# JNP-Solutions/Slacken

Hardware: AMD Instinct MI355X
Metric: classify_throughput_150bp_standard224scale (higher is better)
Workload: dtype u64

## Files before the change

### slacken_amd/csrc/build.hip

```cpp
#include <hip/hip_runtime.h>

#include "engine.h"

namespace slk {

namespace {

constexpr int BW = 4;

__device__ int insert_merge(const TableBuild &t, const int32_t *parents, int32_t ntax, uint64_t key, int32_t taxon, int &max_d) {
  const uint64_t h = fmix64(key);
  if (!shard_keeps(t, h)) return 0;
  uint32_t home;
  uint64_t rem_hi;
  table_slot(t.g, h, home, rem_hi);
  const unsigned long long tmask = (1ULL << t.g.taxon_bits) - 1;
  for (int d = 0; d <= t.disp_limit; d++) {
    unsigned long long *bucket = (unsigned long long *)(t.cells + ((uint64_t)table_bucket(t.g, home, (uint32_t)d) * CELLS));
    const unsigned long long tag = rem_hi | (uint64_t)d;
    const unsigned long long val = (tag << t.g.taxon_bits) | (uint32_t)taxon;
    unsigned long long first = 0;
    for (int c = 0; c < CELLS; c++) {
      unsigned long long cur = __hip_atomic_load(&bucket[c], __ATOMIC_RELAXED, __HIP_MEMORY_SCOPE_AGENT);
      if (cur == 0) {
        unsigned long long old = atomicCAS(&bucket[c], 0ULL, val);
        if (old == 0) {
          max_d = max(max_d, d);
          return 1;
        }
        cur = old;
      }
      if (c == 0) first = cur;
      if (cell_tag(t.g, cur) == tag) {
        for (;;) {
          int32_t old_taxon = (int32_t)(cur & tmask);
          int32_t merged = tax_lca(parents, ntax, old_taxon, taxon);
          if (merged == old_taxon) return 0;
          unsigned long long want = (cur & ~tmask) | (uint32_t)merged;
          unsigned long long prev = atomicCAS(&bucket[c], cur, want);
          if (prev == cur) return 0;
          cur = prev;
        }
      }
    }
    if (t.g.flag && !(first & t.g.flag)) atomicOr(&bucket[0], (unsigned long long)t.g.flag);
  }
  return -1;
}

struct BuildLds {
  uint64_t q_key[BW][128];
  int32_t q_tax[BW][128];
};

__device__ __forceinline__ int code_of(uint32_t c) {
  const uint32_t VM = (1u << 1) | (1u << 3) | (1u << 7) | (1u << 20) | (1u << 21);
  bool ok = ((c & 0xC0) == 0x40) && ((VM >> (c & 31)) & 1);
  uint32_t t = (c >> 1) & 3;
  t ^= t >> 1;
  return ok ? (int)t : 5;
}

__global__ void __launch_bounds__(BW * 64) build_kernel(ScanParams P, TableBuild T, const int32_t *__restrict__ parents,
                                                        int32_t ntax, const uint8_t *__restrict__ bases, uint64_t total_bases,
                                                        const uint64_t *__restrict__ chunk_start,
                                                        const uint32_t *__restrict__ chunk_len,
                                                        const int32_t *__restrict__ chunk_taxon, uint64_t nchunks) {
  extern __shared__ uint64_t ring[];
  __shared__ BuildLds L;
  const uint32_t tid = threadIdx.x, lane = tid & 63;
  const uint32_t wib = __builtin_amdgcn_readfirstlane(tid >> 6);
  const uint32_t stride = BW * 64;
  const int w = P.w, k = P.k, m = P.m;
  const uint64_t c = (uint64_t)blockIdx.x * stride + tid;
  const uint32_t len = c < nchunks ? chunk_len[c] : 0;
  const uint64_t start = c < nchunks ? chunk_start[c] : 0;
  const int32_t taxon = c < nchunks ? chunk_taxon[c] : 0;
  uint32_t maxlen = len;
// ... 151 lines not shown
```

### slacken_amd/csrc/engine.h

```cpp
#pragma once
#include <hip/hip_runtime.h>
#include <stdint.h>

namespace slk {

struct ScanParams {
  int32_t k, m, w;
  int32_t canonical;
  int32_t sh;
  uint64_t xmask;
  uint64_t smask;
  uint64_t keep;
};

constexpr int WIDE_MAXW = 4;
struct WideParams {
  int32_t k, m, w, canonical;
  int32_t W;
  int32_t last_sh;
  uint64_t xmask[WIDE_MAXW];
  uint64_t smask[WIDE_MAXW];
};
struct WideTable {
  uint64_t *keys;
// ... 14 lines not shown
                              const int32_t *span_meta, const uint64_t *out_offsets, void *out, int64_t *out_keys, hipStream_t s);
void launch_wide_probe(const WideTable &t, int W, const uint64_t *offsets, const uint64_t *mate_offsets, uint64_t R,
                       const uint64_t *span_keys, const int32_t *span_meta, const int32_t *span_count, int32_t *span_taxon,
                       hipStream_t s);

#ifndef SLK_BUCKET_CELLS
#define SLK_BUCKET_CELLS 8
#endif
constexpr int CELLS = SLK_BUCKET_CELLS;
constexpr int LPB = CELLS / 2;
constexpr int BUCKET_SHIFT = CELLS == 16 ? 7 : 6;
static_assert(CELLS == 8 || CELLS == 16, "buckets of 64 or 128 bytes");
struct TableGeom {
  uint64_t nbuckets;
  uint64_t rem_mask;
  uint64_t flag;
  int32_t q;
  int32_t taxon_bits;
  int32_t disp_bits;
  int32_t pad;
};
__host__ __device__ __forceinline__ void table_slot(const TableGeom &g, uint64_t h, uint32_t &home, uint64_t &rem_hi) {
  const uint32_t x = (uint32_t)(h >> (64 - g.q));
  const uint64_t prod = (g.nbuckets >> 32) != 0 ? (uint64_t)x << 32 : (uint64_t)x * (uint32_t)g.nbuckets;
  home = (uint32_t)(prod >> g.q);
  const uint64_t extra = (prod & ((1ULL << g.q) - 1)) >= g.nbuckets ? 1 : 0;
  rem_hi = ((h & g.rem_mask) | (extra << (64 - g.q))) << g.disp_bits;
}
__host__ __device__ __forceinline__ uint32_t table_bucket(const TableGeom &g, uint32_t home, uint32_t d) {
  const uint64_t b = (uint64_t)home + d;
  return (uint32_t)(b >= g.nbuckets ? b - g.nbuckets : b);
}
__host__ __device__ __forceinline__ uint64_t cell_tag(const TableGeom &g, uint64_t cell) { return (cell & ~g.flag) >> g.taxon_bits; }
__host__ __device__ inline uint64_t table_hash_of(const TableGeom &g, uint32_t home, uint64_t rem) {
  const uint64_t extra = rem >> (64 - g.q);
  const uint64_t num = (uint64_t)home << g.q;
  const uint64_t x = (num + g.nbuckets - 1) / g.nbuckets + extra;
  return (x << (64 - g.q)) | (rem & g.rem_mask);
}
struct TableView {
  const uint64_t *cells;
  TableGeom g;
  int32_t max_disp;
  const int32_t *to_orig;
};
__device__ __forceinline__ int32_t ext_taxon(const TableView &T, int32_t t) { return (T.to_orig != nullptr && t > 0) ? T.to_orig[t] : t; }

__host__ __device__ inline uint64_t fmix64(uint64_t x) {
  x ^= x >> 33; x *= 0xff51afd7ed558ccdULL;
  x ^= x >> 33; x *= 0xc4ceb9fe1a85ec53ULL;
  x ^= x >> 33;
  return x;
}

__device__ __forceinline__ int32_t tax_parent(const int32_t *parents, int32_t ntax, int32_t t) {
  return ((uint32_t)t < (uint32_t)ntax) ? parents[t] : 0;
}

__device__ inline int32_t tax_lca(const int32_t *parents, int32_t ntax, int32_t a, int32_t b) {
  if (a == 0 || b == 0) return b == 0 ? a : b;
  if (a == b) return a;
  int da = 0, db = 0;
  for (int32_t x = a; x != 0; x = tax_parent(parents, ntax, x)) da++;
  for (int32_t y = b; y != 0; y = tax_parent(parents, ntax, y)) db++;
  for (; da > db; da--) a = tax_parent(parents, ntax, a);
  for (; db > da; db--) b = tax_parent(parents, ntax, b);
// ... 184 lines not shown
```

### slacken_amd/csrc/fused.hip

```cpp
#include "engine.h"

#include <cstdlib>

namespace slk {

constexpr int FW = 4;
constexpr int SPAN_CAP = 128;
constexpr int MAP_CAP = 128;
constexpr int32_t MAP_EMPTY = -1;

struct __attribute__((aligned(16))) RingLds {
  uint32_t fwd_ring[32 + 4];
  uint32_t rc_ring[32 + 4];
};
struct __attribute__((aligned(16))) WaveLds {
  uint64_t span_key[SPAN_CAP];
  int32_t span_meta[SPAN_CAP];
  uint64_t stash[128];
  int32_t result[64];
  int32_t map_key[MAP_CAP];
  int32_t map_cnt[MAP_CAP];
};

__device__ __forceinline__ void wave_sync() {
// ... 130 lines not shown
  int32_t flag = meta_flag(meta);
  bool seq = (lane < cnt) && flag == 1;
  uint64_t h = fmix64(key);
  uint32_t home;
  uint64_t rem_hi;
  table_slot(T.g, h, home, rem_hi);
  ulonglong2 st;
  st.x = home;
  st.y = seq ? rem_hi : NO_TAG;
  ((ulonglong2 *)L->stash)[lane] = st;
  L->result[lane] = 0;
  wave_sync();
  const int g = lane / LPB, c = lane % LPB;
  const uint64_t tmask = (1ULL << T.g.taxon_bits) - 1;
  const uint32_t gmask = (1u << LPB) - 1;
  const char *cellbase = (const char *)T.cells + c * 16;
  uint32_t more = 0;
  {
    ulonglong2 cell[LPB];
#pragma unroll
    for (int s = 0; s < LPB; s++) {
      ulonglong2 e = ((const ulonglong2 *)L->stash)[s * PG + g];
      cell[s] = make_ulonglong2(0, 0);
      if (e.y != NO_TAG) cell[s] = *(const ulonglong2 *)(cellbase + (e.x << BUCKET_SHIFT));
    }
#pragma unroll
    for (int s = 0; s < LPB; s++) {
      const uint64_t want = L->stash[2 * (s * PG + g) + 1];
      const bool act = want != NO_TAG;
      const bool e0 = cell[s].x == 0, e1 = cell[s].y == 0;
      const bool m0 = act && !e0 && cell_tag(T.g, cell[s].x) == want;
      const bool m1 = act && !e1 && cell_tag(T.g, cell[s].y) == want;
      if (m0 || m1) L->result[s * PG + g] = (int32_t)((m0 ? cell[s].x : cell[s].y) & tmask);
      const bool closed = T.g.flag != 0 && c == 0 && (cell[s].x & T.g.flag) == 0;
      const uint64_t B = __ballot(m0 || m1 || e0 || e1 || !act || closed);
      if (((B >> (g * LPB)) & gmask) == 0) more |= 1u << s;
    }
  }
  if (__ballot(more != 0) != 0) {
    for (int d = 1; d <= T.max_disp && __ballot(more != 0) != 0; d++) {
      for (int s = 0; s < LPB; s++) {
        const bool act = (more >> s) & 1;
        ulonglong2 cl = make_ulonglong2(0, 0);
        uint64_t want = 0;
        if (act) {
          ulonglong2 e = ((const ulonglong2 *)L->stash)[s * PG + g];
          want = e.y + (uint64_t)d;
          cl = *(const ulonglong2 *)(cellbase + ((uint64_t)table_bucket(T.g, (uint32_t)e.x, (uint32_t)d) << BUCKET_SHIFT));
        }
        const bool e0 = cl.x == 0, e1 = cl.y == 0;
        const bool m0 = act && !e0 && cell_tag(T.g, cl.x) == want;
        const bool m1 = act && !e1 && cell_tag(T.g, cl.y) == want;
        if (m0 || m1) L->result[s * PG + g] = (int32_t)((m0 ? cl.x : cl.y) & tmask);
        const bool closed = act && T.g.flag != 0 && c == 0 && (cl.x & T.g.flag) == 0;
        const uint64_t B = __ballot(act && (m0 || m1 || e0 || e1 || closed));
        if (act && ((B >> (g * LPB)) & gmask) != 0) more &= ~(1u << s);
      }
    }
  }
  wave_sync();
  int32_t taxon = L->result[lane];
  if (flag == 2) taxon = -1;
  else if (flag == 3) taxon = -2;
  return taxon;
}

__device__ __forceinline__ int char_code2(uint8_t c) {
  uint32_t x = ((uint32_t)(c & 0xDF)) - 0x41;
  switch (x) {
    case 0: return 0;
    case 2: return 1;
    case 6: return 2;
    case 0x13: return 3;
    case 0x14: return 3;
    default: return 5;
  }
}

__device__ int32_t lca_uniform(const int32_t *parents, int32_t ntax, int32_t a, int32_t b) {
  if (a == 0 || b == 0) return b == 0 ? a : b;
  for (int32_t y = b; y != 0; y = ((uint32_t)y < (uint32_t)ntax) ? parents[y] : 0)
    for (int32_t x = a; x != 0; x = ((uint32_t)x < (uint32_t)ntax) ? parents[x] : 0)
      if (x == y) return y;
  return 1;
}

__device__ __forceinline__ uint4 tax_node(const FusedArgs &A, int32_t t) {
// ... 790 lines not shown
```

### slacken_amd/csrc/kernels.hip

```cpp
#include "engine.h"

#include <algorithm>

namespace slk {


__global__ void __launch_bounds__(256) table_insert_kernel(TableBuild t, const int64_t *__restrict__ keys,
                                                           const int32_t *__restrict__ taxa, uint64_t n) {
  uint64_t i = (uint64_t)blockIdx.x * blockDim.x + threadIdx.x;
  uint64_t stride = (uint64_t)gridDim.x * blockDim.x;
  int n_ins = 0, n_dup = 0, n_ovf = 0, max_d = 0;
  for (; i < n; i += stride) {
    int32_t taxon = taxa[i];
    if (taxon == 0) continue;
    uint64_t h = fmix64((uint64_t)keys[i]);
    if (!shard_keeps(t, h)) continue;
    uint32_t home;
    uint64_t rem_hi;
    table_slot(t.g, h, home, rem_hi);
    bool done = false;
    for (int d = 0; d <= t.disp_limit && !done; d++) {
      unsigned long long *bucket = (unsigned long long *)(t.cells + ((uint64_t)table_bucket(t.g, home, (uint32_t)d) * CELLS));
      uint64_t tag = rem_hi | (uint64_t)d;
      unsigned long long val = (tag << t.g.taxon_bits) | (uint32_t)taxon;
      unsigned long long first = 0;
      for (int c = 0; c < CELLS && !done; c++) {
        unsigned long long cur = __hip_atomic_load(&bucket[c], __ATOMIC_RELAXED, __HIP_MEMORY_SCOPE_AGENT);
        if (cur == 0) {
          unsigned long long old = atomicCAS(&bucket[c], 0ULL, val);
          if (old == 0) {
            done = true;
            n_ins++;
            max_d = max(max_d, d);
            break;
          }
          cur = old;
        }
        if (c == 0) first = cur;
        if (cell_tag(t.g, cur) == tag) {
          done = true;
          n_dup++;
        }
      }
      if (!done && t.g.flag && !(first & t.g.flag)) atomicOr(&bucket[0], (unsigned long long)t.g.flag);
    }
    if (!done) n_ovf++;
  }
  for (int o = 32; o > 0; o >>= 1) {
    n_ins += __shfl_xor(n_ins, o);
    n_dup += __shfl_xor(n_dup, o);
    n_ovf += __shfl_xor(n_ovf, o);
    max_d = max(max_d, __shfl_xor(max_d, o));
  }
  if ((threadIdx.x & 63) == 0) {
    if (n_ins) atomicAdd(t.n_inserted, (unsigned long long)n_ins);
    if (n_dup) atomicAdd(t.n_duplicate, (unsigned long long)n_dup);
    if (n_ovf) atomicAdd(t.n_overflow, (unsigned long long)n_ovf);
    if (max_d) atomicMax(t.max_disp, max_d);
  }
}

__device__ __forceinline__ int32_t table_lookup(const TableView &t, uint64_t key) {
  uint64_t h = fmix64(key);
  uint32_t home;
  uint64_t rem_hi;
  table_slot(t.g, h, home, rem_hi);
  uint64_t tmask = (1ULL << t.g.taxon_bits) - 1;
  for (int d = 0; d <= t.max_disp; d++) {
    const ulonglong2 *b = (const ulonglong2 *)(t.cells + ((uint64_t)table_bucket(t.g, home, (uint32_t)d) * CELLS));
    uint64_t tag = rem_hi | (uint64_t)d;
    uint64_t cells[CELLS];
#pragma unroll
    for (int c = 0; c < LPB; c++) { ulonglong2 v = b[c]; cells[2 * c] = v.x; cells[2 * c + 1] = v.y; }
    bool has_empty = false;
    int32_t found = 0;
#pragma unroll
    for (int c = 0; c < CELLS; c++) {
      has_empty |= (cells[c] == 0);
      if (cells[c] != 0 && cell_tag(t.g, cells[c]) == tag) found = (int32_t)(cells[c] & tmask);
    }
    if (found) return found;
    if (has_empty) return 0;
    if (t.g.flag && !(cells[0] & t.g.flag)) return 0;
  }
  return 0;
}

__global__ void __launch_bounds__(256) table_lookup_kernel(TableView t, const int64_t *__restrict__ keys, uint64_t n,
                                                           int32_t *__restrict__ out) {
  uint64_t i = (uint64_t)blockIdx.x * blockDim.x + threadIdx.x;
  uint64_t stride = (uint64_t)gridDim.x * blockDim.x;
  for (; i < n; i += stride) out[i] = ext_taxon(t, table_lookup(t, (uint64_t)keys[i]));
}


__device__ __forceinline__ int char_code(uint8_t c) {
  if (c == '\n' || c == '\r') return 4;
  switch (c | 0x20) {
    case 'a': return 0;
    case 'c': return 1;
    case 'g': return 2;
    case 't': return 3;
    case 'u': return 3;
    default: return 5;
  }
}

struct SpanWriter {
  uint64_t *keys;
  int32_t *meta;
  uint64_t base;
  int32_t n;
  bool first;
  bool have_last;
  uint64_t last;

// ... 602 lines not shown
```

### slacken_amd/csrc/lane.hip

```cpp
#include "engine.h"

#include <algorithm>
#include <cstddef>
#include <cstdio>
#include <cstdlib>

namespace slk {

#ifndef SLK_LANE_LW
#define SLK_LANE_LW 4
#endif
constexpr int LW = SLK_LANE_LW;
constexpr int QCAP = 128;
#ifndef SLK_SBLK
#define SLK_SBLK 5
#endif
constexpr int SBLK = SLK_SBLK;
#ifndef SLK_OMAP
#define SLK_OMAP 12
#endif
constexpr int OMAP = SLK_OMAP;
constexpr int OMAP_CNT_BITS = 10;
constexpr uint32_t OMAP_CNT_MASK = (1u << OMAP_CNT_BITS) - 1;

struct __attribute__((aligned(16))) LaneLds {
  uint64_t q_key[QCAP];
  uint32_t q_meta[QCAP];
  uint64_t stash[128];
  uint32_t found[64];
  uint4 sbuf[(SBLK - 1) * 64];
  uint32_t omap[OMAP * 64];
  uint32_t o_flags[64];
  uint64_t rb[64];
  uint16_t q_ord[QCAP];
};

#ifdef SLK_TUNING
#define SLK_TUNE(...) __VA_ARGS__
#define SLK_TUNE_ON(bit) ((dbg & (bit)) != 0)
#else
#define SLK_TUNE(...)
#define SLK_TUNE_ON(bit) false
#endif

#ifndef SLK_PROBE_NT
#define SLK_PROBE_NT 0
#endif
__device__ __forceinline__ ulonglong2 SLK_PROBE_LOAD(const ulonglong2 *p) {
#if SLK_PROBE_NT
  ulonglong2 v;
  v.x = __builtin_nontemporal_load(&p->x);
  v.y = __builtin_nontemporal_load(&p->y);
  return v;
#else
  return *p;
#endif
}

__device__ __forceinline__ void lane_wave_sync() {
  __builtin_amdgcn_fence(__ATOMIC_RELEASE, "wavefront");
  __builtin_amdgcn_wave_barrier();
  __builtin_amdgcn_fence(__ATOMIC_ACQUIRE, "wavefront");
}
__device__ __forceinline__ uint64_t lmin64(uint64_t a, uint64_t b) { return a < b ? a : b; }

template <bool LONG>
__device__ __forceinline__ void fold_hit(LaneLds *L, uint32_t *ocnt, bool in, uint32_t meta, int32_t taxon) {
  if (in && taxon != 0) {
    const int owner = meta & 63;
    const int32_t kmers = (int32_t)((meta >> 7) & 0x1FFF);
    if (meta & 64) atomicAdd(&L->o_flags[owner], 1u);
    uint32_t slot = (uint32_t)(((uint64_t)((uint32_t)taxon * 0x9E3779B1u) * (uint32_t)OMAP) >> 32);
    int p = 0;
    if (LONG) {
      for (; p < OMAP; p++) {
// ... 19 lines not shown
__device__ __forceinline__ int probe_batch(LaneLds *L, uint32_t *ocnt, const TableView &T, int qhead, int qn, int cnt, int lane, int dbg,
                                           int32_t *hit_meta, int32_t *hit_taxon) {
  const uint64_t NO_TAG = ~0ULL;
  const bool in = lane < cnt;
  const int qi = (qhead + lane) & (QCAP - 1);
  const uint64_t key = L->q_key[qi];
  const uint32_t meta = L->q_meta[qi];
  const uint32_t ord = HITS ? L->q_ord[qi] : 0u;
  const uint64_t h = fmix64(key);
  uint32_t home;
  uint64_t rem_hi;
  table_slot(T.g, h, home, rem_hi);
  uint4 st;
  const uint32_t disp = (meta >> 20) & 255;
  st.x = table_bucket(T.g, home, disp);
  st.y = 0;
  const uint64_t tag = in ? (rem_hi + disp) : NO_TAG;
  st.z = (uint32_t)tag; st.w = (uint32_t)(tag >> 32);
  ((uint4 *)L->stash)[lane] = st;
  L->found[lane] = 0;
  lane_wave_sync();
  const int g = lane / LPB, c = lane % LPB;
  const uint64_t tmask = (1ULL << T.g.taxon_bits) - 1;
  const char *cellbase = (const char *)T.cells + c * 16;
  ulonglong2 cell[LPB];
#pragma unroll
  for (int s = 0; s < LPB; s++) {
    uint32_t bkt = ((const uint4 *)L->stash)[s * PG + g].x;
    SLK_TUNE(if (dbg & 4) bkt &= 1023u;)
    cell[s] = SLK_PROBE_LOAD((const ulonglong2 *)(cellbase + ((uint64_t)bkt << BUCKET_SHIFT)));
  }
  constexpr uint64_t GROUP_LSB = LPB == 4 ? 0x1111111111111111ULL : 0x0101010101010101ULL;
  int requeued = 0;
#pragma unroll
  for (int s = 0; s < LPB; s++) {
    const uint2 tg = *(const uint2 *)&((const uint4 *)L->stash)[s * PG + g].z;
    const uint64_t want = ((uint64_t)tg.y << 32) | tg.x;
    const bool act = want != NO_TAG;
    const bool e0 = cell[s].x == 0, e1 = cell[s].y == 0;
    const bool m0 = act && !e0 && cell_tag(T.g, cell[s].x) == want;
    const bool m1 = act && !e1 && cell_tag(T.g, cell[s].y) == want;
    if (m0 || m1) L->found[s * PG + g] = (uint32_t)((m0 ? cell[s].x : cell[s].y) & tmask);
    const bool closed = T.g.flag != 0 && c == 0 && (cell[s].x & T.g.flag) == 0;
    const uint64_t B = __ballot(m0 || m1 || e0 || e1 || !act || closed);
    uint64_t any = B;
#pragma unroll
    for (int i = 1; i < LPB; i <<= 1) any |= any >> i;
    if ((any & GROUP_LSB) != GROUP_LSB) {
      const int qj = (qhead + s * PG + g) & (QCAP - 1);
      const uint32_t m_old = L->q_meta[qj];
      const bool again = c == 0 && ((B >> (g * LPB)) & ((1u << LPB) - 1)) == 0 && (int)((m_old >> 20) & 255) < T.max_disp;
      const uint64_t k_old = L->q_key[qj];
      const uint16_t o_old = HITS ? L->q_ord[qj] : (uint16_t)0;
      const uint64_t R = __ballot(again);
      lane_wave_sync();
      if (again) {
        const int slot = (qhead + qn + requeued + __builtin_amdgcn_mbcnt_hi((uint32_t)(R >> 32), __builtin_amdgcn_mbcnt_lo((uint32_t)R, 0))) & (QCAP - 1);
        L->q_key[slot] = k_old;
        L->q_meta[slot] = m_old + (1u << 20);
        if (HITS) L->q_ord[slot] = o_old;
      }
      requeued += __popcll(R);
    }
  }
  lane_wave_sync();
  const int32_t taxon = (int32_t)L->found[lane];
  if (!SLK_TUNE_ON(2)) fold_hit<LONG>(L, ocnt, in, meta, taxon);
  if (HITS && in) {
    const uint64_t at = L->rb[meta & 63] + ord;
    hit_taxon[at] = ext_taxon(T, taxon);
    hit_meta[at] = pack_meta((int32_t)((meta >> 7) & 0x1FFF), 1, (meta >> 6) & 1);
  }
  lane_wave_sync();
  return requeued;
}

#ifndef SLK_STREAM_NT
#define SLK_STREAM_NT 0
#endif
#ifndef SLK_APPLY_ROWS
#define SLK_APPLY_ROWS 4
#endif
template <class T> __device__ __forceinline__ T SLK_STREAM_LOAD(const T *p) {
#if SLK_STREAM_NT
  return __builtin_nontemporal_load(p);
#else
  return *p;
#endif
}
template <class T> __device__ __forceinline__ void SLK_STREAM_STORE(T *p, T v) {
#if SLK_STREAM_NT
  __builtin_nontemporal_store(v, p);
#else
  *p = v;
#endif
}

__device__ __forceinline__ uint64_t lane_readlane64(uint64_t v, int src) {
  uint32_t lo = __builtin_amdgcn_readlane((uint32_t)v, src), hi = __builtin_amdgcn_readlane((uint32_t)(v >> 32), src);
// ... 12 lines not shown
  if (base >= S.side_n) return;
  const uint64_t i = base + (uint64_t)lane;
  const bool in = i < S.side_n;
  const uint64_t h = fmix64(key);
  uint32_t home;
  uint64_t rem_hi;
  table_slot(T.g, h, home, rem_hi);
  const uint64_t tag = in ? rem_hi : ~0ULL;
  uint4 st;
  st.x = home; st.y = 0; st.z = (uint32_t)tag; st.w = (uint32_t)(tag >> 32);
  ((uint4 *)L->stash)[lane] = st;
  L->found[lane] = 0;
  lane_wave_sync();
  const int g = lane / LPB, c = lane % LPB;
  const uint64_t tmask = (1ULL << T.g.taxon_bits) - 1;
  const char *cellbase = (const char *)T.cells + c * 16;
  ulonglong2 cell[LPB];
#pragma unroll
  for (int s = 0; s < LPB; s++) {
    uint32_t bkt = ((const uint4 *)L->stash)[s * PG + g].x;
    SLK_TUNE(if (dbg & 4) bkt &= 1023u;)
    cell[s] = SLK_PROBE_LOAD((const ulonglong2 *)(cellbase + ((uint64_t)bkt << BUCKET_SHIFT)));
  }
  uint32_t unresolved = 0;
#pragma unroll
  for (int s = 0; s < LPB; s++) {
    const uint2 tg = *(const uint2 *)&((const uint4 *)L->stash)[s * PG + g].z;
    const uint64_t want = ((uint64_t)tg.y << 32) | tg.x;
    const bool act = want != ~0ULL;
    const bool e0 = cell[s].x == 0, e1 = cell[s].y == 0;
    const bool m0 = act && !e0 && cell_tag(T.g, cell[s].x) == want;
    const bool m1 = act && !e1 && cell_tag(T.g, cell[s].y) == want;
    if (m0 || m1) L->found[s * PG + g] = (uint32_t)((m0 ? cell[s].x : cell[s].y) & tmask);
    const bool closed = T.g.flag != 0 && c == 0 && (cell[s].x & T.g.flag) == 0;
    const uint64_t B = __ballot(m0 || m1 || e0 || e1 || !act || closed);
    if (((B >> (g * LPB)) & ((1u << LPB) - 1)) == 0) unresolved |= 1u << s;
  }
  lane_wave_sync();
  int32_t taxon = (int32_t)L->found[lane];
  const uint32_t ur = (uint32_t)__shfl((int)unresolved, (lane % PG) * LPB);
  if (in && ((ur >> (lane / PG)) & 1)) {
    for (int d = 1; d <= T.max_disp; d++) {
      const ulonglong2 *b = (const ulonglong2 *)(T.cells + ((uint64_t)table_bucket(T.g, home, (uint32_t)d) * CELLS));
      const uint64_t want = rem_hi | (uint64_t)d;
      bool has_empty = false, closed = false;
      int32_t hit = 0;
#pragma unroll
      for (int q = 0; q < LPB; q++) {
        const ulonglong2 v = b[q];
        has_empty |= (v.x == 0) | (v.y == 0);
        if (q == 0) closed = T.g.flag != 0 && (v.x & T.g.flag) == 0;
        if (v.x != 0 && cell_tag(T.g, v.x) == want) hit = (int32_t)(v.x & tmask);
        if (v.y != 0 && cell_tag(T.g, v.y) == want) hit = (int32_t)(v.y & tmask);
      }
      if (hit) { taxon = hit; break; }
      if (has_empty || closed) break;
    }
  }
  if (in && !SLK_TUNE_ON(128)) SLK_STREAM_STORE(&S.side_out[i], ext_taxon(T, taxon));
  lane_wave_sync();
}

template <bool HITS>
__device__ __forceinline__ void apply_rows(LaneLds *L, const ApplyJob &J, int lane, uint64_t row0, uint32_t nrows) {
  const uint32_t ns = (uint32_t)J.n_shards;
  constexpr int U = SLK_APPLY_ROWS;
  for (uint32_t b = 0; b < nrows; b += U) {
    uint64_t at[U];
    bool in[U];
#pragma unroll
    for (int u = 0; u < U; u++) {
      in[u] = false;
      at[u] = 0;
      if (b + u < nrows) {
        uint32_t off = 0;
        for (uint32_t sh = 0; sh < ns; sh++) {
          const uint4 e = J.batch_log[(row0 + b + u) * ns + sh];
          const uint32_t cnt = e.z;
          if (cnt == 0) continue;
          if ((uint32_t)lane >= off && (uint32_t)lane < off + cnt) {
            in[u] = true;
            const uint32_t i = (uint32_t)lane - off;
            at[u] = (uint64_t)sh * J.cap + (i < e.w ? e.x + i : e.y + (i - e.w));
          }
// ... 194 lines not shown
        uint64_t len = A.offsets[r + 1] - A.offsets[r];
        if (A.mate_offsets) len += A.mate_offsets[r + 1] - A.mate_offsets[r];
        route[j] = len <= 1000 ? (int)HandOn::SHORT : route_by_length(len, A.long_max, A.long_bound[0], A.long_bound[1], A.long_bound[2],
                                                                      A.seg_min_len, A.wave_min, A.wave_ratio_q10);
        rank[j] = atomicAdd(&cnt[route[j]], 1u);
      }
    }
    __syncthreads();
    if (threadIdx.x < NL && cnt[threadIdx.x] != 0)
      base[threadIdx.x] = atomicAdd(&A.hand_hdr[HandOn::count_word((int)threadIdx.x)], (unsigned long long)cnt[threadIdx.x]);
    if (threadIdx.x == 0) {
      uint32_t handed = 0;
      for (int l = 0; l < NL; l++) if (l != HandOn::SHORT) handed += cnt[l];
      if (handed) atomicAdd(&A.hand_hdr[HandOn::HANDED], (unsigned long long)handed);
    }
    __syncthreads();
#pragma unroll
    for (int j = 0; j < PER; j++)
      if (route[j] >= 0)
        A.hand_lists[HandOn::list_at(route[j], A.hand_stride, A.hand_long_cap) + base[route[j]] + rank[j]] =
            (uint32_t)(c * chunk + (uint64_t)j * 256 + threadIdx.x);
    __syncthreads();
  }
}
void launch_route(const FusedArgs &A, hipStream_t s) {
  if (A.R == 0) return;
  hipLaunchKernelGGL(route_kernel, dim3((unsigned)std::min<uint64_t>((A.R + 2047) / 2048, 2048)), dim3(256), 0, s, A);
}

template <bool HITS, bool LONG>
__device__ __forceinline__ void resolve_lane(LaneLds *L, uint32_t *ocnt, const FusedArgs &A, int lane, uint64_t r, uint32_t oflags, int32_t total,
                                             int32_t nhits, int32_t np, int dbg) {
  const int32_t nd = (int32_t)oflags;
  uint32_t *const ecnt = LONG ? ocnt : L->omap;
  int D = 0;
  for (int s = 0; s < OMAP; s++) {
    const uint32_t e = L->omap[s * 64 + lane];
    if (e != 0) {
      if (LONG) ocnt[D * 64 + lane] = ocnt[s * 64 + lane];
      L->omap[D * 64 + lane] = e;
      D++;
    }
  }
#define ENT_TAXON(j) (LONG ? (int32_t)L->omap[(j) * 64 + lane] : (int32_t)(L->omap[(j) * 64 + lane] >> OMAP_CNT_BITS))
#define ENT_COUNT(j) (LONG ? (int32_t)ecnt[(j) * 64 + lane] : (int32_t)(ecnt[(j) * 64 + lane] & OMAP_CNT_MASK))
  int32_t maxTaxon = D ? ENT_TAXON(0) : 0;
  const int32_t c0 = D ? ENT_COUNT(0) : 0;
  uint32_t *const tin = (uint32_t *)L, *const tout = tin + OMAP * 64;
  static_assert(offsetof(LaneLds, omap) >= 2 * OMAP * 64 * sizeof(uint32_t), "the intervals alias the queue and the read stream's slots");
  uint32_t m_in = 0, m_out = 0;
  int32_t sum_all = c0;
  if (D >= 2 && !SLK_TUNE_ON(16)) {
#pragma unroll
    for (int j = 0; j < OMAP; j++) {
      if (j < D) {
        const uint4 nj = lane_node(A.nodes, A.ntax, ENT_TAXON(j));
        tin[j * 64 + lane] = nj.y;
        tout[j * 64 + lane] = nj.z;
      }
    }
    maxTaxon = 0;
    sum_all = 0;
    int32_t best = 0;
    for (int a = 0; a < D; a++) {
      const uint32_t ain = tin[a * 64 + lane], aout = tout[a * 64 + lane];
      int32_t score = 0;
      for (int b = 0; b < D; b++)
        score += (tin[b * 64 + lane] <= ain && ain <= tout[b * 64 + lane]) ? ENT_COUNT(b) : 0;
      sum_all += ENT_COUNT(a);
      if (score > best) {
        maxTaxon = ENT_TAXON(a); best = score; m_in = ain; m_out = aout;
      } else if (score == best) {
        if (m_in <= ain && ain <= m_out) {
        } else if (ain <= m_in && m_in <= aout) {
          maxTaxon = ENT_TAXON(a); m_in = ain; m_out = aout;
        } else {
          int32_t x = (int32_t)lane_node(A.nodes, A.ntax, maxTaxon).x;
          uint4 nx = make_uint4(0, 0, 0, 0);
          while (x != 0) {
            nx = lane_node(A.nodes, A.ntax, x);
            if (nx.y <= ain && ain <= nx.z) break;
            x = (int32_t)nx.x;
          }
          if (x == 0) { x = 1; nx = lane_node(A.nodes, A.ntax, 1); }
          maxTaxon = x; m_in = nx.y; m_out = nx.z;
        }
      }
    }
  }
  for (int32_t c = 0; c < A.C; c++) {
    const double required = ceil(__dmul_rn(A.thr.v[c], (double)total));
    int32_t mt = maxTaxon;
    if (D < 2 || SLK_TUNE_ON(16)) {
      if ((double)c0 < required) mt = 0;
    } else {
      uint32_t cin = m_in, cout = m_out;
      uint4 cur = make_uint4(0, 0, 0, 0);
      bool have_cur = false;
      while (mt != 0) {
        int32_t ms = 0;
        bool side = false;
        int up = -1;
        uint32_t up_in = 0;
        for (int j = 0; j < D; j++) {
          const uint32_t jin = tin[j * 64 + lane], jout = tout[j * 64 + lane];
          const bool inside = cin <= jin && jin <= cout;
          ms += inside ? ENT_COUNT(j) : 0;
          const bool above = !inside && jin <= cin && cin <= jout;
          side = side || (!inside && !above);
          if (above && (up < 0 || jin > up_in)) { up = j; up_in = jin; }
        }
        if ((double)ms >= required) break;
        if (ms == sum_all) { mt = 0; break; }
        if (!side) {
          mt = ENT_TAXON(up); cin = up_in; cout = tout[up * 64 + lane];
          have_cur = false;
        } else {
          if (!have_cur) cur = lane_node(A.nodes, A.ntax, mt);
          mt = (int32_t)cur.x;
          if (mt != 0) { cur = lane_node(A.nodes, A.ntax, mt); have_cur = true; cin = cur.y; cout = cur.z; }
        }
      }
    }
    bool classified = (mt != 0) && (nd >= A.min_hit_groups);
    A.out_taxon[(uint64_t)c * A.out_stride + r] = classified ? ext_taxon(A.T, mt) : 0;
    A.out_classified[(uint64_t)c * A.out_stride + r] = classified ? 1 : 0;
  }
#undef ENT_TAXON
#undef ENT_COUNT
  if (A.out_nd) A.out_nd[r] = nd;
  if (A.out_tk) A.out_tk[r] = total;
  if (A.out_nh) A.out_nh[r] = nhits;
  if (HITS) A.span_count[r] = nhits;
  if (A.out_np) A.out_np[r] = np;
}

template <bool W5, int MODE, bool HITS, bool LONG>
__device__ __forceinline__ void lane_body(const FusedArgs &A, const ShardIO &S, const ApplyJob *Jp, int32_t *defer, uint32_t max_len, int dbg) {
  extern __shared__ __attribute__((aligned(16))) unsigned char lds_raw[];
  const int lane = threadIdx.x & 63;
  const int wib = __builtin_amdgcn_readfirstlane(threadIdx.x >> 6);
  const ScanParams P = A.P;
  const int k = P.k, m = P.m, w = P.w;
  const size_t fixed = HITS ? sizeof(LaneLds) : offsetof(LaneLds, rb);
  const size_t win_bytes = W5 ? 0 : (size_t)w * 64 * sizeof(uint64_t);
  const size_t per_wave = fixed + win_bytes + (LONG ? (size_t)OMAP * 64 * sizeof(uint32_t) : 0);
  LaneLds *L = (LaneLds *)(lds_raw + (size_t)wib * per_wave);
  uint64_t *win = (uint64_t *)((unsigned char *)L + fixed);
  uint32_t *ocnt = LONG ? (uint32_t *)((unsigned char *)L + fixed + win_bytes) : nullptr;
  const bool paired = A.mate_bases != nullptr;
  const bool scans = MODE != LANE_EMIT || A.R != 0;
  const uint64_t bases_end = scans ? A.offsets[A.R] : 0, mates_end = (scans && paired) ? A.mate_offsets[A.R] : 0;
  uint64_t cls_n[5] = {0, 0, 0, 0, 0}, cls_tiles[5] = {0, 0, 0, 0, 0};
  uint64_t ntiles = (A.R + 63) / 64;
  if (LONG) {
    ntiles = 0;
#pragma unroll
    for (int c = 0; c < 5; c++) {
      cls_n[c] = c == 0 ? (A.route_first ? A.hand_hdr[HandOn::N_SHORT] : 0ULL) : A.hand_hdr[c - 1];
      cls_tiles[c] = (cls_n[c] + 63) / 64;
      ntiles += cls_tiles[c];
    }
  }
  const uint64_t nwaves = (uint64_t)gridDim.x * LW;
  const uint64_t etiles = ntiles;
  const uint64_t atiles = MODE == LANE_EMIT ? (Jp->A.R + 63) / 64 : 0;
  if (MODE == LANE_EMIT) ntiles = max(etiles, atiles);
// ... 333 lines not shown
      for (uint32_t i = p0 + (uint32_t)lane; i < p1; i += 64) S.send_keys[(uint64_t)sh * S.cap + i] = 0;
    }
  }
}

template <bool W5, int MODE, bool HITS, bool LONG>
__global__ void LANE_BOUNDS lane_kernel(FusedArgs A, ShardIO S, int32_t *defer, uint32_t max_len, int dbg) {
  lane_body<W5, MODE, HITS, LONG>(A, S, nullptr, defer, max_len, dbg);
}
template <bool W5, bool HITS>
__global__ void LANE_BOUNDS lane_step_kernel(FusedArgs A, ShardIO S, ApplyJob J, int32_t *defer, uint32_t max_len, int dbg) {
  lane_body<W5, LANE_EMIT, HITS, false>(A, S, &J, defer, max_len, dbg);
}

static size_t lane_lds_per_wave(bool hits, bool w5, int w, bool lng) {
  return (hits ? sizeof(LaneLds) : offsetof(LaneLds, rb)) + (w5 ? 0 : (size_t)w * 64 * sizeof(uint64_t)) + (lng ? (size_t)OMAP * 64 * sizeof(uint32_t) : 0);
}

template <bool HITS, bool LONG>
static void launch_lane_mode(const FusedArgs &A, int32_t *defer, uint32_t max_len, hipStream_t s) {
  if (A.R == 0) return;
  const bool w5 = A.P.w == 5;
  const size_t per_wave = lane_lds_per_wave(HITS, w5, A.P.w, LONG);
  static const int extra_lds = getenv("SLK_LANE_EXTRA_LDS") ? atoi(getenv("SLK_LANE_EXTRA_LDS")) : 0;
  size_t lds = per_wave * LW + (size_t)extra_lds;
  uint64_t tiles = (A.R + 63) / 64;
  uint64_t blocks = (tiles + LW - 1) / LW;
  static const int bpc = getenv("SLK_LANE_BLOCKS_PER_CU") ? atoi(getenv("SLK_LANE_BLOCKS_PER_CU")) : 0;
  if (bpc > 0 && blocks > (uint64_t)256 * bpc) blocks = (uint64_t)256 * bpc;
  if (LONG && blocks > 256 * 5) blocks = 256 * 5;
  dim3 g((unsigned)blocks), b(LW * 64);
#ifdef SLK_TUNING
  static const int dbg = getenv("SLK_DEBUG_ABLATE") ? atoi(getenv("SLK_DEBUG_ABLATE")) : 0;
#else
  const int dbg = 0;
#endif
  static bool occ_printed = false;
  if (getenv("SLK_DEBUG_OCC") && !occ_printed) {
    occ_printed = true;
    int nb = 0;
    (void)hipOccupancyMaxActiveBlocksPerMultiprocessor(&nb, w5 ? (const void *)lane_kernel<true, LANE_LOCAL, HITS, LONG> : (const void *)lane_kernel<false, LANE_LOCAL, HITS, LONG>, LW * 64, lds);
    fprintf(stderr, "[slk] lane kernel: %zu B LDS per block, %d blocks (%d waves) resident per CU\n", lds, nb, nb * LW);
  }
  if (w5) hipLaunchKernelGGL((lane_kernel<true, LANE_LOCAL, HITS, LONG>), g, b, lds, s, A, ShardIO{}, defer, max_len, dbg);
  else hipLaunchKernelGGL((lane_kernel<false, LANE_LOCAL, HITS, LONG>), g, b, lds, s, A, ShardIO{}, defer, max_len, dbg);
}

void launch_lane(const FusedArgs &A, int32_t *defer, uint32_t max_len, hipStream_t s) {
  if (A.span_taxon) launch_lane_mode<true, false>(A, defer, max_len, s);
  else launch_lane_mode<false, false>(A, defer, max_len, s);
}
void launch_lane_long(const FusedArgs &A, uint32_t max_len, hipStream_t s) {
  if (A.span_taxon) launch_lane_mode<true, true>(A, nullptr, max_len, s);
  else launch_lane_mode<false, true>(A, nullptr, max_len, s);
}

template <bool W5, bool HITS>
static void launch_step_mode(const FusedArgs &A, const ShardIO &S, const ApplyJob &J, int32_t *defer, uint32_t max_len, hipStream_t s) {
  const uint64_t tiles = std::max((A.R + 63) / 64, (J.A.R + 63) / 64);
  if (tiles == 0) return;
  const size_t lds = lane_lds_per_wave(HITS, W5, A.P.w, false) * LW;
  static int resident[2][2] = {{0, 0}, {0, 0}};
  static int cus = 0;
  if (cus == 0) {
    int dev = 0;
    (void)hipGetDevice(&dev);
    if (hipDeviceGetAttribute(&cus, hipDeviceAttributeMultiprocessorCount, dev) != hipSuccess || cus <= 0) cus = 256;
  }
  int nb = W5 ? resident[1][HITS] : 0;
  if (nb == 0) {
    if (hipOccupancyMaxActiveBlocksPerMultiprocessor(&nb, (const void *)lane_step_kernel<W5, HITS>, LW * 64, lds) != hipSuccess || nb <= 0) nb = 4;
    if (W5) resident[1][HITS] = nb;
  }
  static const int bpc = getenv("SLK_STEP_BLOCKS_PER_CU") ? atoi(getenv("SLK_STEP_BLOCKS_PER_CU")) : 0;
  if (bpc > 0) nb = bpc;
  const uint64_t blocks = std::min<uint64_t>((tiles + LW - 1) / LW, (uint64_t)cus * nb);
#ifdef SLK_TUNING
  static const int dbg = getenv("SLK_DEBUG_ABLATE") ? atoi(getenv("SLK_DEBUG_ABLATE")) : 0;
// ... 13 lines not shown
```

### slacken_amd/csrc/shard.hip

```cpp
#include <hip/hip_runtime.h>

#include "engine.h"

#include <cstdlib>

namespace slk {

namespace {

constexpr int SW = 4;

__device__ __forceinline__ void wsync() {
  __builtin_amdgcn_fence(__ATOMIC_RELEASE, "wavefront");
  __builtin_amdgcn_wave_barrier();
  __builtin_amdgcn_fence(__ATOMIC_ACQUIRE, "wavefront");
}

__global__ void __launch_bounds__(SW * 64) lookup_coop_kernel(TableView T, const int64_t *__restrict__ keys, uint64_t n,
                                                              int32_t *__restrict__ out) {
  constexpr int PG = 64 / LPB;
  __shared__ __attribute__((aligned(16))) uint4 stash_all[SW][64];
  const int lane = threadIdx.x & 63;
  const int wib = __builtin_amdgcn_readfirstlane(threadIdx.x >> 6);
  uint4 *stash = stash_all[wib];
// ... 1 lines not shown
  const uint64_t tmask = (1ULL << T.g.taxon_bits) - 1;
  const int g = lane / LPB, c = lane % LPB;
  const char *cellbase = (const char *)T.cells + c * 16;
  const uint64_t units = (n + 63) / 64;
  for (uint64_t unit = (uint64_t)blockIdx.x * SW + wib; unit < units; unit += nwaves) {
    const uint64_t base = unit * 64;
    const uint64_t i = base + lane;
    const bool in = i < n;
    const uint64_t key = in ? (uint64_t)keys[i] : 0;
    const uint64_t h = fmix64(key);
    uint32_t home;
    uint64_t rem_hi;
    table_slot(T.g, h, home, rem_hi);
    const uint64_t tag = in ? rem_hi : ~0ULL;
    uint4 st;
    st.x = home;
    st.y = 0;
    st.z = (uint32_t)tag;
    st.w = (uint32_t)(tag >> 32);
    stash[lane] = st;
    wsync();
    ulonglong2 cell[LPB];
#pragma unroll
    for (int s = 0; s < LPB; s++) cell[s] = *(const ulonglong2 *)(cellbase + ((uint64_t)stash[s * PG + g].x << BUCKET_SHIFT));
    uint32_t unresolved = 0;
#pragma unroll
    for (int s = 0; s < LPB; s++) {
      const uint64_t want = ((uint64_t)stash[s * PG + g].w << 32) | stash[s * PG + g].z;
      const bool act = want != ~0ULL;
      const bool e0 = cell[s].x == 0, e1 = cell[s].y == 0;
      const bool m0 = act && !e0 && cell_tag(T.g, cell[s].x) == want;
      const bool m1 = act && !e1 && cell_tag(T.g, cell[s].y) == want;
      if (m0 || m1) stash[s * PG + g].y = (uint32_t)((m0 ? cell[s].x : cell[s].y) & tmask);
      const bool closed = T.g.flag != 0 && c == 0 && (cell[s].x & T.g.flag) == 0;
      const uint64_t B = __ballot(m0 || m1 || e0 || e1 || !act || closed);
      if (((B >> (g * LPB)) & ((1u << LPB) - 1)) == 0) unresolved |= 1u << s;
    }
    wsync();
    int32_t taxon = (int32_t)stash[lane].y;
    const uint32_t ur = (uint32_t)__shfl((int)unresolved, (lane % PG) * LPB);
    if (in && ((ur >> (lane / PG)) & 1)) {
      for (int d = 1; d <= T.max_disp; d++) {
        const ulonglong2 *b = (const ulonglong2 *)(T.cells + ((uint64_t)table_bucket(T.g, home, (uint32_t)d) * CELLS));
        const uint64_t want = rem_hi | (uint64_t)d;
        bool has_empty = false, closed = false;
        int32_t found = 0;
#pragma unroll
        for (int q = 0; q < LPB; q++) {
          ulonglong2 v = b[q];
          has_empty |= (v.x == 0) | (v.y == 0);
          if (q == 0) closed = T.g.flag != 0 && (v.x & T.g.flag) == 0;
          if (v.x != 0 && cell_tag(T.g, v.x) == want) found = (int32_t)(v.x & tmask);
          if (v.y != 0 && cell_tag(T.g, v.y) == want) found = (int32_t)(v.y & tmask);
        }
        if (found) { taxon = found; break; }
        if (has_empty || closed) break;
      }
    }
    if (in) out[i] = ext_taxon(T, taxon);
    wsync();
  }
}

}

void launch_lookup_coop(const TableView &t, const int64_t *keys, uint64_t n, int32_t *out, hipStream_t s) {
  if (n == 0) return;
  static const int bpc = getenv("SLK_LOOKUP_BLOCKS_PER_CU") ? std::max(1, atoi(getenv("SLK_LOOKUP_BLOCKS_PER_CU"))) : 16;
  uint64_t blocks = std::min<uint64_t>((n + SW * 64 - 1) / (SW * 64), (uint64_t)256 * bpc);
  hipLaunchKernelGGL(lookup_coop_kernel, dim3((unsigned)blocks), dim3(SW * 64), 0, s, t, keys, n, out);
}
}
```

Before: 1158.

## Spread bucket overflow flags across cells by tag fingerprint

Replaces the single per-bucket overflow flag in cell 0 with a flag in a cell chosen by a fingerprint of the key's tag. Build paths set the flag on that cell and every lookup path checks the matching cell, so a bucket is 'closed' only for the subset of tags whose fingerprint cell carries no overflow flag. This lets more lookups of absent keys stop at the home bucket instead of probing displaced buckets. It also adds tuning-only counters under SLK_TUNING. The table must be rebuilt with the new layout, and there is a small per-probe cost for the fingerprint computation.

```diff
diff --git a/slacken_amd/csrc/build.hip b/slacken_amd/csrc/build.hip
--- a/slacken_amd/csrc/build.hip
+++ b/slacken_amd/csrc/build.hip
@@ -15,11 +15,12 @@
   uint64_t rem_hi;
   table_slot(t.g, h, home, rem_hi);
   const unsigned long long tmask = (1ULL << t.g.taxon_bits) - 1;
+  const int fp = table_fp(t.g, rem_hi);
   for (int d = 0; d <= t.disp_limit; d++) {
     unsigned long long *bucket = (unsigned long long *)(t.cells + ((uint64_t)table_bucket(t.g, home, (uint32_t)d) * CELLS));
     const unsigned long long tag = rem_hi | (uint64_t)d;
     const unsigned long long val = (tag << t.g.taxon_bits) | (uint32_t)taxon;
-    unsigned long long first = 0;
+    unsigned long long fpcell = 0;
     for (int c = 0; c < CELLS; c++) {
       unsigned long long cur = __hip_atomic_load(&bucket[c], __ATOMIC_RELAXED, __HIP_MEMORY_SCOPE_AGENT);
       if (cur == 0) {
@@ -30,7 +31,7 @@
         }
         cur = old;
       }
-      if (c == 0) first = cur;
+      if (c == fp) fpcell = cur;
       if (cell_tag(t.g, cur) == tag) {
         for (;;) {
           int32_t old_taxon = (int32_t)(cur & tmask);
@@ -43,7 +44,7 @@
         }
       }
     }
-    if (t.g.flag && !(first & t.g.flag)) atomicOr(&bucket[0], (unsigned long long)t.g.flag);
+    if (t.g.flag && !(fpcell & t.g.flag)) atomicOr(&bucket[fp], (unsigned long long)t.g.flag);
   }
   return -1;
 }
diff --git a/slacken_amd/csrc/engine.h b/slacken_amd/csrc/engine.h
--- a/slacken_amd/csrc/engine.h
+++ b/slacken_amd/csrc/engine.h
@@ -70,6 +70,11 @@
   return (uint32_t)(b >= g.nbuckets ? b - g.nbuckets : b);
 }
 __host__ __device__ __forceinline__ uint64_t cell_tag(const TableGeom &g, uint64_t cell) { return (cell & ~g.flag) >> g.taxon_bits; }
+__host__ __device__ __forceinline__ int table_fp(const TableGeom &g, uint64_t tag) { return (int)((tag >> g.disp_bits) & (CELLS - 1)); }
+__host__ __device__ __forceinline__ bool bucket_closed(const TableGeom &g, uint64_t tag, int c, ulonglong2 v) {
+  const int fp = table_fp(g, tag);
+  return g.flag != 0 && c == (fp >> 1) && (((fp & 1) ? v.y : v.x) & g.flag) == 0;
+}
 __host__ __device__ inline uint64_t table_hash_of(const TableGeom &g, uint32_t home, uint64_t rem) {
   const uint64_t extra = rem >> (64 - g.q);
   const uint64_t num = (uint64_t)home << g.q;
diff --git a/slacken_amd/csrc/fused.hip b/slacken_amd/csrc/fused.hip
--- a/slacken_amd/csrc/fused.hip
+++ b/slacken_amd/csrc/fused.hip
@@ -186,7 +186,7 @@
       const bool m0 = act && !e0 && cell_tag(T.g, cell[s].x) == want;
       const bool m1 = act && !e1 && cell_tag(T.g, cell[s].y) == want;
       if (m0 || m1) L->result[s * PG + g] = (int32_t)((m0 ? cell[s].x : cell[s].y) & tmask);
-      const bool closed = T.g.flag != 0 && c == 0 && (cell[s].x & T.g.flag) == 0;
+      const bool closed = bucket_closed(T.g, want, c, cell[s]);
       const uint64_t B = __ballot(m0 || m1 || e0 || e1 || !act || closed);
       if (((B >> (g * LPB)) & gmask) == 0) more |= 1u << s;
     }
@@ -206,7 +206,7 @@
         const bool m0 = act && !e0 && cell_tag(T.g, cl.x) == want;
         const bool m1 = act && !e1 && cell_tag(T.g, cl.y) == want;
         if (m0 || m1) L->result[s * PG + g] = (int32_t)((m0 ? cl.x : cl.y) & tmask);
-        const bool closed = act && T.g.flag != 0 && c == 0 && (cl.x & T.g.flag) == 0;
+        const bool closed = act && bucket_closed(T.g, want, c, cl);
         const uint64_t B = __ballot(act && (m0 || m1 || e0 || e1 || closed));
         if (act && ((B >> (g * LPB)) & gmask) != 0) more &= ~(1u << s);
       }
diff --git a/slacken_amd/csrc/kernels.hip b/slacken_amd/csrc/kernels.hip
--- a/slacken_amd/csrc/kernels.hip
+++ b/slacken_amd/csrc/kernels.hip
@@ -18,12 +18,13 @@
     uint32_t home;
     uint64_t rem_hi;
     table_slot(t.g, h, home, rem_hi);
+    const int fp = table_fp(t.g, rem_hi);
     bool done = false;
     for (int d = 0; d <= t.disp_limit && !done; d++) {
       unsigned long long *bucket = (unsigned long long *)(t.cells + ((uint64_t)table_bucket(t.g, home, (uint32_t)d) * CELLS));
       uint64_t tag = rem_hi | (uint64_t)d;
       unsigned long long val = (tag << t.g.taxon_bits) | (uint32_t)taxon;
-      unsigned long long first = 0;
+      unsigned long long fpcell = 0;
       for (int c = 0; c < CELLS && !done; c++) {
         unsigned long long cur = __hip_atomic_load(&bucket[c], __ATOMIC_RELAXED, __HIP_MEMORY_SCOPE_AGENT);
         if (cur == 0) {
@@ -36,13 +37,13 @@
           }
           cur = old;
         }
-        if (c == 0) first = cur;
+        if (c == fp) fpcell = cur;
         if (cell_tag(t.g, cur) == tag) {
           done = true;
           n_dup++;
         }
       }
-      if (!done && t.g.flag && !(first & t.g.flag)) atomicOr(&bucket[0], (unsigned long long)t.g.flag);
+      if (!done && t.g.flag && !(fpcell & t.g.flag)) atomicOr(&bucket[fp], (unsigned long long)t.g.flag);
     }
     if (!done) n_ovf++;
   }
@@ -66,6 +67,7 @@
   uint64_t rem_hi;
   table_slot(t.g, h, home, rem_hi);
   uint64_t tmask = (1ULL << t.g.taxon_bits) - 1;
+  const int fp = table_fp(t.g, rem_hi);
   for (int d = 0; d <= t.max_disp; d++) {
     const ulonglong2 *b = (const ulonglong2 *)(t.cells + ((uint64_t)table_bucket(t.g, home, (uint32_t)d) * CELLS));
     uint64_t tag = rem_hi | (uint64_t)d;
@@ -74,14 +76,16 @@
     for (int c = 0; c < LPB; c++) { ulonglong2 v = b[c]; cells[2 * c] = v.x; cells[2 * c + 1] = v.y; }
     bool has_empty = false;
     int32_t found = 0;
+    uint64_t fpcell = 0;
 #pragma unroll
     for (int c = 0; c < CELLS; c++) {
       has_empty |= (cells[c] == 0);
+      if (c == fp) fpcell = cells[c];
       if (cells[c] != 0 && cell_tag(t.g, cells[c]) == tag) found = (int32_t)(cells[c] & tmask);
     }
     if (found) return found;
     if (has_empty) return 0;
-    if (t.g.flag && !(cells[0] & t.g.flag)) return 0;
+    if (t.g.flag && !(fpcell & t.g.flag)) return 0;
   }
   return 0;
 }
diff --git a/slacken_amd/csrc/lane.hip b/slacken_amd/csrc/lane.hip
--- a/slacken_amd/csrc/lane.hip
+++ b/slacken_amd/csrc/lane.hip
@@ -41,6 +41,13 @@
 #else
 #define SLK_TUNE(...)
 #define SLK_TUNE_ON(bit) false
+#endif
+#ifdef SLK_TUNING
+enum { TC_FIRST, TC_SECOND, TC_SECOND_ABSENT, TC_SECOND_DISPLACED, TC_NODE, TC_OUT_BYTES, TC_N };
+__device__ unsigned long long tune_count[TC_N];
+#define SLK_COUNT(i, n) do { if (SLK_TUNE_ON(1024) && (n) != 0) atomicAdd(&tune_count[i], (unsigned long long)(n)); } while (0)
+#else
+#define SLK_COUNT(i, n) do {} while (0)
 #endif
 
 #ifndef SLK_PROBE_NT
@@ -126,6 +133,7 @@
   }
   constexpr uint64_t GROUP_LSB = LPB == 4 ? 0x1111111111111111ULL : 0x0101010101010101ULL;
   int requeued = 0;
+  SLK_TUNE(uint64_t rq = 0;)
 #pragma unroll
   for (int s = 0; s < LPB; s++) {
     const uint2 tg = *(const uint2 *)&((const uint4 *)L->stash)[s * PG + g].z;
@@ -135,7 +143,7 @@
     const bool m0 = act && !e0 && cell_tag(T.g, cell[s].x) == want;
     const bool m1 = act && !e1 && cell_tag(T.g, cell[s].y) == want;
     if (m0 || m1) L->found[s * PG + g] = (uint32_t)((m0 ? cell[s].x : cell[s].y) & tmask);
-    const bool closed = T.g.flag != 0 && c == 0 && (cell[s].x & T.g.flag) == 0;
+    const bool closed = bucket_closed(T.g, want, c, cell[s]);
     const uint64_t B = __ballot(m0 || m1 || e0 || e1 || !act || closed);
     uint64_t any = B;
 #pragma unroll
@@ -155,10 +163,16 @@
         if (HITS) L->q_ord[slot] = o_old;
       }
       requeued += __popcll(R);
+      SLK_TUNE(for (uint64_t x = R; x != 0; x &= x - 1) rq |= 1ULL << (s * PG + __builtin_ctzll(x) / LPB);)
     }
   }
   lane_wave_sync();
   const int32_t taxon = (int32_t)L->found[lane];
+  SLK_TUNE(if (in) {
+    const uint32_t d = (meta >> 20) & 255;
+    SLK_COUNT(d ? TC_SECOND : TC_FIRST, 1);
+    if (d != 0 && ((rq >> lane) & 1) == 0) SLK_COUNT(taxon != 0 ? TC_SECOND_DISPLACED : TC_SECOND_ABSENT, d);
+  })
   if (!SLK_TUNE_ON(2)) fold_hit<LONG>(L, ocnt, in, meta, taxon);
   if (HITS && in) {
     const uint64_t at = L->rb[meta & 63] + ord;
@@ -237,7 +251,7 @@
     const bool m0 = act && !e0 && cell_tag(T.g, cell[s].x) == want;
     const bool m1 = act && !e1 && cell_tag(T.g, cell[s].y) == want;
     if (m0 || m1) L->found[s * PG + g] = (uint32_t)((m0 ? cell[s].x : cell[s].y) & tmask);
-    const bool closed = T.g.flag != 0 && c == 0 && (cell[s].x & T.g.flag) == 0;
+    const bool closed = bucket_closed(T.g, want, c, cell[s]);
     const uint64_t B = __ballot(m0 || m1 || e0 || e1 || !act || closed);
     if (((B >> (g * LPB)) & ((1u << LPB) - 1)) == 0) unresolved |= 1u << s;
   }
@@ -254,7 +268,7 @@
       for (int q = 0; q < LPB; q++) {
         const ulonglong2 v = b[q];
         has_empty |= (v.x == 0) | (v.y == 0);
-        if (q == 0) closed = T.g.flag != 0 && (v.x & T.g.flag) == 0;
+        closed |= bucket_closed(T.g, want, q, v);
         if (v.x != 0 && cell_tag(T.g, v.x) == want) hit = (int32_t)(v.x & tmask);
         if (v.y != 0 && cell_tag(T.g, v.y) == want) hit = (int32_t)(v.y & tmask);
       }
@@ -515,6 +529,8 @@
 __device__ __forceinline__ void resolve_lane(LaneLds *L, uint32_t *ocnt, const FusedArgs &A, int lane, uint64_t r, uint32_t oflags, int32_t total,
                                              int32_t nhits, int32_t np, int dbg) {
   const int32_t nd = (int32_t)oflags;
+  SLK_TUNE(uint32_t n_node = 0;)
+  auto node = [&](int32_t t) { SLK_TUNE(n_node++;) return lane_node(A.nodes, A.ntax, t); };
   uint32_t *const ecnt = LONG ? ocnt : L->omap;
   int D = 0;
   for (int s = 0; s < OMAP; s++) {
@@ -537,7 +553,7 @@
 #pragma unroll
     for (int j = 0; j < OMAP; j++) {
       if (j < D) {
-        const uint4 nj = lane_node(A.nodes, A.ntax, ENT_TAXON(j));
+        const uint4 nj = node(ENT_TAXON(j));
         tin[j * 64 + lane] = nj.y;
         tout[j * 64 + lane] = nj.z;
       }
@@ -558,14 +574,14 @@
         } else if (ain <= m_in && m_in <= aout) {
           maxTaxon = ENT_TAXON(a); m_in = ain; m_out = aout;
         } else {
-          int32_t x = (int32_t)lane_node(A.nodes, A.ntax, maxTaxon).x;
+          int32_t x = (int32_t)node(maxTaxon).x;
           uint4 nx = make_uint4(0, 0, 0, 0);
           while (x != 0) {
-            nx = lane_node(A.nodes, A.ntax, x);
+            nx = node(x);
             if (nx.y <= ain && ain <= nx.z) break;
             x = (int32_t)nx.x;
           }
-          if (x == 0) { x = 1; nx = lane_node(A.nodes, A.ntax, 1); }
+          if (x == 0) { x = 1; nx = node(1); }
           maxTaxon = x; m_in = nx.y; m_out = nx.z;
         }
       }
@@ -599,23 +615,27 @@
           mt = ENT_TAXON(up); cin = up_in; cout = tout[up * 64 + lane];
           have_cur = false;
         } else {
-          if (!have_cur) cur = lane_node(A.nodes, A.ntax, mt);
+          if (!have_cur) cur = node(mt);
           mt = (int32_t)cur.x;
-          if (mt != 0) { cur = lane_node(A.nodes, A.ntax, mt); have_cur = true; cin = cur.y; cout = cur.z; }
+          if (mt != 0) { cur = node(mt); have_cur = true; cin = cur.y; cout = cur.z; }
         }
       }
     }
     bool classified = (mt != 0) && (nd >= A.min_hit_groups);
+    SLK_TUNE(if (dbg & 512) continue;)
     A.out_taxon[(uint64_t)c * A.out_stride + r] = classified ? ext_taxon(A.T, mt) : 0;
     A.out_classified[(uint64_t)c * A.out_stride + r] = classified ? 1 : 0;
   }
 #undef ENT_TAXON
 #undef ENT_COUNT
+  SLK_TUNE(if (dbg & 512) return;)
   if (A.out_nd) A.out_nd[r] = nd;
   if (A.out_tk) A.out_tk[r] = total;
   if (A.out_nh) A.out_nh[r] = nhits;
   if (HITS) A.span_count[r] = nhits;
   if (A.out_np) A.out_np[r] = np;
+  SLK_COUNT(TC_NODE, n_node);
+  SLK_COUNT(TC_OUT_BYTES, 5 * A.C + 4 * ((A.out_nd != nullptr) + (A.out_tk != nullptr) + (A.out_nh != nullptr) + HITS + (A.out_np != nullptr)));
 }
 
 template <bool W5, int MODE, bool HITS, bool LONG>
@@ -1015,6 +1035,10 @@
   dim3 g((unsigned)blocks), b(LW * 64);
 #ifdef SLK_TUNING
   static const int dbg = getenv("SLK_DEBUG_ABLATE") ? atoi(getenv("SLK_DEBUG_ABLATE")) : 0;
+  if (dbg & 1024) {
+    static const unsigned long long zero[TC_N] = {};
+    (void)hipMemcpyToSymbolAsync(HIP_SYMBOL(tune_count), zero, sizeof zero, 0, hipMemcpyHostToDevice, s);
+  }
 #else
   const int dbg = 0;
 #endif
@@ -1027,6 +1051,16 @@
   }
   if (w5) hipLaunchKernelGGL((lane_kernel<true, LANE_LOCAL, HITS, LONG>), g, b, lds, s, A, ShardIO{}, defer, max_len, dbg);
   else hipLaunchKernelGGL((lane_kernel<false, LANE_LOCAL, HITS, LONG>), g, b, lds, s, A, ShardIO{}, defer, max_len, dbg);
+#ifdef SLK_TUNING
+  if (dbg & 1024) {
+    unsigned long long c[TC_N];
+    (void)hipStreamSynchronize(s);
+    (void)hipMemcpyFromSymbol(c, HIP_SYMBOL(tune_count), sizeof c, 0, hipMemcpyDeviceToHost);
+    fprintf(stderr, "[slk-tune] lane_kernel<%d,0,%d,%d> R=%llu first_probes=%llu second_probes=%llu second_absent=%llu "
+            "second_displaced=%llu node_loads=%llu out_bytes=%llu\n", (int)w5, (int)HITS, (int)LONG, (unsigned long long)A.R,
+            c[TC_FIRST], c[TC_SECOND], c[TC_SECOND_ABSENT], c[TC_SECOND_DISPLACED], c[TC_NODE], c[TC_OUT_BYTES]);
+  }
+#endif
 }
 
 void launch_lane(const FusedArgs &A, int32_t *defer, uint32_t max_len, hipStream_t s) {
diff --git a/slacken_amd/csrc/shard.hip b/slacken_amd/csrc/shard.hip
--- a/slacken_amd/csrc/shard.hip
+++ b/slacken_amd/csrc/shard.hip
@@ -57,7 +57,7 @@
       const bool m0 = act && !e0 && cell_tag(T.g, cell[s].x) == want;
       const bool m1 = act && !e1 && cell_tag(T.g, cell[s].y) == want;
       if (m0 || m1) stash[s * PG + g].y = (uint32_t)((m0 ? cell[s].x : cell[s].y) & tmask);
-      const bool closed = T.g.flag != 0 && c == 0 && (cell[s].x & T.g.flag) == 0;
+      const bool closed = bucket_closed(T.g, want, c, cell[s]);
       const uint64_t B = __ballot(m0 || m1 || e0 || e1 || !act || closed);
       if (((B >> (g * LPB)) & ((1u << LPB) - 1)) == 0) unresolved |= 1u << s;
     }
@@ -74,7 +74,7 @@
         for (int q = 0; q < LPB; q++) {
           ulonglong2 v = b[q];
           has_empty |= (v.x == 0) | (v.y == 0);
-          if (q == 0) closed = T.g.flag != 0 && (v.x & T.g.flag) == 0;
+          closed |= bucket_closed(T.g, want, q, v);
           if (v.x != 0 && cell_tag(T.g, v.x) == want) found = (int32_t)(v.x & tmask);
           if (v.y != 0 && cell_tag(T.g, v.y) == want) found = (int32_t)(v.y & tmask);
         }
```

Result: no change. 1169, median of 6 (+1.0%).
